# fatlipp/eacham

Measured on AMD Instinct MI355X. Metric: image-pairs matched/s + BA iters/s, 200-frame/50k-landmark synthetic, higher is better.
Workload: dtype i8; 1 GPU; S200 matching: 200 frames x 2000 kpts x 256-D, 19900 unordered pairs (both directions + mutual check); pairs_per_rank=19900, parallelism=pairs sharded over 1 GPU(s)

## Files before the change

### eacham_amd/csrc/context.hip

```cpp
#include "context.hpp"
#include <algorithm>

#include <cstdlib>
#include <cstring>
#include <dlfcn.h>
#include <new>

namespace eacham {

int ensure_workspace(eacham_ctx* ctx, size_t bytes) {
    if (bytes <= ctx->ws_bytes) return EACHAM_OK;
    if (ctx->ws) {
        EACHAM_HIP_TRY(ctx, hipStreamSynchronize(ctx->stream));
        EACHAM_HIP_TRY(ctx, hipFree(ctx->ws));
        ctx->ws = nullptr;
        ctx->ws_bytes = 0;
    }
    EACHAM_HIP_TRY(ctx, hipMalloc(&ctx->ws, bytes));
    ctx->ws_bytes = bytes;
    return EACHAM_OK;
}

int ensure_io(eacham_ctx* ctx, size_t bytes) {
    if (bytes <= ctx->io_bytes) return EACHAM_OK;
// ... 94 lines not shown
    f.dim = dim;
    f.ks = ks;
    f.ntiles = ntiles;
    ctx->ks_common = ks;
    ctx->kind_common = kind;
    ctx->wide_bytes_common = wide_bytes;
    ctx->frame_table_dirty = true;
    ctx->bits_table_dirty = true;
}

__global__ void gather_tiles_kernel(const FrameDev* __restrict__ frames, int n, int* __restrict__ used) {
    const int i = blockIdx.x * blockDim.x + threadIdx.x;
    if (i < n) used[i] = frames[i].meta ? frames[i].meta[1] : frames[i].ntiles;
}

int sync_frame_table(eacham_ctx* ctx) {
    if (!ctx->frame_table_dirty) return EACHAM_OK;
    int need = (int)ctx->frames.size();
    if (need + 1 > ctx->frame_table_cap) {
        if (ctx->frame_table_dev) {
            EACHAM_HIP_TRY(ctx, hipStreamSynchronize(ctx->stream));
            EACHAM_HIP_TRY(ctx, hipFree(ctx->frame_table_dev));
            ctx->frame_table_dev = nullptr;
        }
        int cap = need < 64 ? 64 : need * 2;
        EACHAM_HIP_TRY(ctx, hipMalloc((void**)&ctx->frame_table_dev, sizeof(FrameDev) * cap));
        ctx->frame_table_cap = cap;
    }
    std::vector<FrameDev> tab(need + 1);
    {
        FrameDev& e = tab[need];
        e.frag = nullptr; e.norm = nullptr; e.normb = nullptr; e.screen = nullptr;
        e.orig = ctx->flag_dev->standin_rows; e.pos = ctx->flag_dev->standin_rows; e.meta = ctx->flag_dev->standin_meta;
        e.n = 0; e.ntiles = 0; e.resident = 1;
    }
    for (int i = 0; i < need; ++i) {
        const FrameHost& f = ctx->frames[i];
        tab[i].frag = f.frag;
        tab[i].norm = f.norm;
        tab[i].normb = f.normb;
        tab[i].orig = f.orig;
        tab[i].pos = f.pos;
        tab[i].meta = f.meta;
        tab[i].screen = f.screen;
        tab[i].n = f.n < 0 ? 0 : f.n;
        tab[i].ntiles = f.n < 0 ? 0 : f.ntiles;
        tab[i].resident = f.n < 0 ? 0 : 1;
    }
    {
        EACHAM_HIP_TRY(ctx, hipMemcpyAsync(ctx->frame_table_dev, tab.data(), sizeof(FrameDev) * (need + 1),
                                           hipMemcpyHostToDevice, ctx->stream));
        int* used_dev = nullptr;
        if (need == 0) {
            ctx->frame_table_dirty = false;
            return EACHAM_OK;
        }
        EACHAM_HIP_TRY(ctx, hipMalloc((void**)&used_dev, sizeof(int) * need));
        gather_tiles_kernel<<<(need + 255) / 256, 256, 0, ctx->stream>>>(ctx->frame_table_dev, need, used_dev);
        std::vector<int> used(need);
        hipError_t e = hipMemcpyAsync(used.data(), used_dev, sizeof(int) * need, hipMemcpyDeviceToHost, ctx->stream);
        if (e == hipSuccess) e = hipStreamSynchronize(ctx->stream);
        (void)hipFree(used_dev);
        EACHAM_HIP_TRY(ctx, e);
        for (int i = 0; i < need; ++i) ctx->frames[i].tiles_used = used[i];
    }
    ctx->frame_table_dirty = false;
    return EACHAM_OK;
}

namespace {
typedef int (*roctx_push_t)(const char*);
typedef int (*roctx_pop_t)(void);
roctx_push_t g_roctx_push = nullptr;
roctx_pop_t g_roctx_pop = nullptr;
// ... 173 lines not shown
int eacham_clear_descriptors(eacham_ctx* ctx) {
    if (!ctx) return EACHAM_ERR_INVALID;
    std::lock_guard<std::mutex> lock(ctx->mu);
    (void)hipSetDevice(ctx->device);
    EACHAM_HIP_TRY(ctx, hipStreamSynchronize(ctx->stream));
    for (auto& f : ctx->frames) release_frame(f);
    ctx->frames.clear();
    ctx->ks_common = 0;
    ctx->kind_common = FRAME_INT8;
    ctx->wide_bytes_common = 0;
    ctx->frame_table_dirty = true;
    ctx->bits_table_dirty = true;
    return EACHAM_OK;
}

void eacham_ctx_destroy(eacham_ctx* ctx) {
    if (!ctx) return;
    (void)hipSetDevice(ctx->device);
    (void)hipStreamSynchronize(ctx->stream);
    for (auto& f : ctx->frames) release_frame(f);
    if (ctx->table16_dev) (void)hipFree(ctx->table16_dev);
    if (ctx->bits_table_dev) (void)hipFree((void*)ctx->bits_table_dev);
    if (ctx->frame_table_dev) (void)hipFree(ctx->frame_table_dev);
    if (ctx->flag_dev) (void)hipFree(ctx->flag_dev);
    if (ctx->pairs_safe) (void)hipFree(ctx->pairs_safe);
    if (ctx->ws) (void)hipFree(ctx->ws);
    if (ctx->io) (void)hipFree(ctx->io);
    if (ctx->io_host) (void)hipHostFree(ctx->io_host);
    for (auto& b : ctx->ba_pool) {
        if (b.dev) (void)hipFree(b.dev);
        if (b.pinned) (void)hipHostFree(b.pinned);
    }
    for (auto& sc : ctx->ba_scratch)
        if (sc.dev) (void)hipFree(sc.dev);
    for (auto& s : ctx->prof)
        for (auto& ev : s.events) {
            (void)hipEventDestroy(ev.first);
            (void)hipEventDestroy(ev.second);
        }
    for (hipEvent_t e : {ctx->ev_tile[0], ctx->ev_tile[1], ctx->ev_fin[0], ctx->ev_fin[1], ctx->ev_join})
        if (e) (void)hipEventDestroy(e);
    if (ctx->stream2) (void)hipStreamDestroy(ctx->stream2);
    (void)hipStreamDestroy(ctx->stream);
    delete ctx;
}

// ... 51 lines not shown
```

### eacham_amd/csrc/context.hpp

```cpp
#pragma once

#include <hip/hip_runtime.h>

#include <algorithm>
#include <cstdarg>
#include <cstddef>
#include <cstring>
#include <cstdint>
#include <cstdio>
#include <mutex>
#include <string>
#include <utility>
#include <vector>

#include "../../include/eacham_hip.h"
#include "io_layout.hpp"

namespace eacham {

enum FrameKind {
    FRAME_INT8 = 0,
    FRAME_F32 = 1,
    FRAME_BITS = 2,
    FRAME_BITS_WIDE = 3,
// ... 9 lines not shown
    int pad1[4];
    unsigned long long dot16[6];
    unsigned long long screen[3];
    int pad2[6];
};
static_assert(offsetof(FlagBlock, bad_pair) == 1 * sizeof(int) && offsetof(FlagBlock, standin_meta) == 8 * sizeof(int) &&
                  offsetof(FlagBlock, standin_rows) == 16 * sizeof(int) && offsetof(FlagBlock, colprune) == 32 * sizeof(int) &&
                  offsetof(FlagBlock, dot16) == 40 * sizeof(int) && offsetof(FlagBlock, screen) == 52 * sizeof(int) &&
                  sizeof(FlagBlock) == 64 * sizeof(int),
              "the block's words stay where the kernels and the debug calls have always found them");

struct FrameDev {
    const int4* frag;
    const int* norm;
    const int* normb;
    const int* orig;
    const int* pos;
    const int* meta;
    const int4* screen;
    int n;
    int ntiles;
    int resident;
};

struct FrameHost {
    int4* frag = nullptr;
    int* norm = nullptr;
    int* normb = nullptr;
    int* orig = nullptr;
    int* pos = nullptr;
    int* meta = nullptr;
    int4* screen = nullptr;
    unsigned* bits = nullptr;
    int n = -1;
    int dim = 0;
    int ks = 0;
    int ntiles = 0;
    int tiles_used = 0;
    void* img16 = nullptr;
    bool img16_ready = false;
    bool img16_bad = false;
    float img16_maxn = 0.0f;
};

struct BaBlock {
    void* dev = nullptr;
// ... 7 lines not shown
    size_t bytes = 0;
};

struct ProfileSlot {
    std::vector<std::pair<hipEvent_t, hipEvent_t>> events;
    size_t used = 0;
    int64_t launches = 0;
    double total_ms = 0.0;
};

}

struct eacham_ctx {
    int device = 0;
    hipStream_t stream = nullptr;
    hipStream_t stream2 = nullptr;
    hipEvent_t ev_tile[2] = {nullptr, nullptr}, ev_fin[2] = {nullptr, nullptr}, ev_join = nullptr;
    std::mutex mu;
    std::string err;

    std::vector<eacham::FrameHost> frames;
    eacham::FrameDev* frame_table_dev = nullptr;
    int frame_table_cap = 0;
    bool frame_table_dirty = true;
    eacham::FlagBlock* flag_dev = nullptr;
    int ks_common = 0;
    eacham::FrameKind kind_common = eacham::FRAME_INT8;
    const unsigned** bits_table_dev = nullptr;
    int bits_table_cap = 0;
    bool bits_table_dirty = true;
    int wide_bytes_common = 0;
    size_t wide_budget_bytes = 0;
    long long wide_debug[4] = {0, 0, 0, 0};
    void* table16_dev = nullptr;
    int table16_cap = 0;
    long long dot16_fallback_pairs = 0;

    void* ws = nullptr;
    size_t ws_bytes = 0;
    int2* pairs_safe = nullptr;
    int pairs_safe_cap = 0;
    void* io = nullptr;
    size_t io_bytes = 0;
    void* io_host = nullptr;
    size_t io_host_bytes = 0;

// ... 158 lines not shown
    }
};
struct LmedsLaunch {
    int kind, P;
    long long S, max_n;
    int score_grid;
    const long long *point_ptr, *sample_ptr;
    const double *a, *b, *K;
    bool has_K;
    const int* sample_idx;
    double* cand_models;
    int *n_models, *first, *sample_problem, *total, *scan_ws;
    float *cand_medians, *rows;
    double* models;
    float *medians, *thresholds;
    int* inliers;
    unsigned char* masks;
    int *winner, *n_candidates;
};
int lmeds_score_grid(long long cand_cap, long long max_n);
bool lmeds_needs_rows(long long max_n);
int lmeds_launch(eacham_ctx* ctx, hipStream_t st, const LmedsLaunch& L);
int sync_frame_table(eacham_ctx* ctx);
int sanitize_pairs(eacham_ctx* ctx, const int2* pairs_dev, int npairs, const int2** out);

int open_frame_slot(eacham_ctx* ctx, int frame_id, FrameKind kind, int n, int max_rows, int ks, int wide_bytes, FrameHost** slot);
void release_frame(FrameHost& f);
void commit_frame(eacham_ctx* ctx, FrameHost& f, FrameKind kind, int n, int dim, int ks, int ntiles, int wide_bytes);

int upload_frame_f32(eacham_ctx* ctx, int frame_id, const float* src_dev, int n, int dim);
int run_match_f32(eacham_ctx* ctx, const int2* pairs_dev, int npairs, double ratio, int min_dir, int min_mutual, int mode,
                  int* counts_dev, long long* offsets_dev, uint2* edges_dev, long long edge_cap, long long* total_dev,
                  int4* stats_dev);
struct MatchPlanF32 {
    int row_stride, wb_stride, wgs_per_pair;
    int batch;
    size_t off_rowres, off_colpart, off_matches, total;
};
MatchPlanF32 plan_match_f32(const eacham_ctx* ctx, int npairs);
int run_match_dot(eacham_ctx* ctx, const int2* pairs_dev, int npairs, float min_score, int min_dir, int min_mutual, int mode,
                  int* counts_dev, long long* offsets_dev, uint2* edges_dev, float* scores_dev, long long edge_cap,
                  long long* total_dev, int4* stats_dev);
void launch_match_tile_dot(eacham_ctx* ctx, const int2* pb, int nb, const MatchPlanF32& pl, int2* rr, int2* cp);
int launch_match_dot_tail(eacham_ctx* ctx, const MatchPlanF32& pl, const int2* pb, int nb, int first, bool is_last, int2* rr, int2* cp,
                          float min_score, int min_dir, int min_mutual, int mode, int* counts_dev, long long* offsets_dev,
                          uint2* edges_dev, float* scores_dev, long long edge_cap, long long* total_dev, int4* stats_dev);
// ... 30 lines not shown
```

### eacham_amd/csrc/matcher.hip

```cpp
#include "context.hpp"
#include "match_screen.hpp"
#include "match_tail.hpp"

#include <algorithm>
#include <climits>
#include <cstdlib>
#include <type_traits>

namespace eacham {

typedef int v4i __attribute__((ext_vector_type(4)));
typedef int v16i __attribute__((ext_vector_type(16)));
typedef const v4i __attribute__((address_space(1)))* gfrag_t;
typedef const int __attribute__((address_space(1)))* gint_t;

constexpr int PADH = 8350000;
constexpr int KEY_SHIFT = 7;
constexpr int KEY_MASK = (1 << KEY_SHIFT) - 1;
constexpr int CHUNK_TILES = 1 << KEY_SHIFT;
constexpr int MAX_ROWS = 16384;
constexpr int WG_THREADS = 256;
constexpr int WAVES = WG_THREADS / 64;
constexpr int MATCH_NSUB = 2;
constexpr int ROWS_PER_WAVE = 32 * MATCH_NSUB;
// ... 119 lines not shown
            const int x = min(max((int)src[(size_t)row * dim + k], 0), 255);
            code = screen::encode(x);
            const int m = screen::decode(code), d = x - screen::reconstruct(code);
            m2 += m * m;
            err += d * d;
        }
        codes[e] = (unsigned char)code;
    }
    uint32_t w[6];
    screen::pack32(codes, w);
    char* tb = image + (size_t)tile * SCREEN_TILE_BYTES + ks * SCREEN_STEP_BYTES;
    const int lane = 32 * h + r;
    *reinterpret_cast<v4i*>(tb + 16 * lane) = v4i{(int)w[0], (int)w[1], (int)w[2], (int)w[3]};
    *reinterpret_cast<int2*>(tb + 1024 + 8 * lane) = make_int2((int)w[4], (int)w[5]);
    if (m2) atomicAdd(&msq[j], m2);
    if (err) atomicAdd(&sr[j], err);
}
__global__ void finish_screen_kernel(int npad, const int* __restrict__ orig, int* __restrict__ msq, const int* __restrict__ sr, int* __restrict__ eb) {
    const int j = blockIdx.x * blockDim.x + threadIdx.x;
    if (j >= npad) return;
    const bool real_row = orig[j] >= 0;
    reinterpret_cast<float*>(msq)[j] = real_row ? 0.5f * (float)msq[j] : SCREEN_PAD;
    if (real_row) atomicMax(eb, sr[j]);
}

__device__ __forceinline__ unsigned vmed3(unsigned a, unsigned b, unsigned c) {
    unsigned d;
    asm("v_med3_u32 %0, %1, %2, %3" : "=v"(d) : "v"(a), "v"(b), "v"(c));
    return d;
}
__device__ __forceinline__ unsigned umin(unsigned a, unsigned b) { return a < b ? a : b; }
__device__ __forceinline__ unsigned umax(unsigned a, unsigned b) { return a > b ? a : b; }


__device__ __forceinline__ unsigned lds_addr(const void* p) {
    return (unsigned)(unsigned long long)(const __attribute__((address_space(3))) void*)p;
}
template <class V>
__device__ __forceinline__ void lds_read_frag(V& dst, unsigned addr, int offset_bytes) {
    asm volatile("ds_read_b128 %0, %1 offset:%2" : "=v"(dst) : "v"(addr), "n"(offset_bytes));
}

template <int KS>
__global__ __launch_bounds__(WG_THREADS, 2) void match_tile_kernel(
    const FrameDev* __restrict__ frames, const int2* __restrict__ pairs, int wgs_per_pair, int col_chunks,
    uint4* __restrict__ rowres, uint2* __restrict__ colpart, int wb_stride, int row_stride) {
// ... 543 lines not shown
        }
    }
}

typedef int v2i __attribute__((ext_vector_type(2)));
typedef int v6i __attribute__((ext_vector_type(6)));
typedef int v8i __attribute__((ext_vector_type(8)));
typedef float v4f __attribute__((ext_vector_type(4)));
typedef float v16f __attribute__((ext_vector_type(16)));
__device__ __forceinline__ void lds_read_frag64(v2i& dst, unsigned addr, int offset_bytes) {
    asm volatile("ds_read_b64 %0, %1 offset:%2" : "=v"(dst) : "v"(addr), "n"(offset_bytes));
}
__device__ __forceinline__ float fmin3(float a, float b, float c) {
    float d;
    asm("v_min3_f32 %0, %1, %2, %3" : "=v"(d) : "v"(a), "v"(b), "v"(c));
    return d;
}
template <int METRIC>
__device__ __forceinline__ bool ratio_pass(int d2_best, int d2_second, double ratio);
struct ScreenFrag { v4i lo; v2i hi; };
__device__ __forceinline__ v8i screen_operand(const ScreenFrag& f) { return v8i{f.lo[0], f.lo[1], f.lo[2], f.lo[3], f.hi[0], f.hi[1], 0, 0}; }

template <int METRIC>
__global__ __launch_bounds__(WG_THREADS, 3) void match_screen_kernel(const FrameDev* __restrict__ frames, const int2* __restrict__ pairs,
                                                                     int wgs_per_pair, uint4* __restrict__ rowres, int row_stride, double ratio,
                                                                     unsigned long long* __restrict__ openmask, int mask_stride) {
    constexpr int NSUB = 2, KS = SCREEN_KS;
    constexpr int TILE_V4 = SCREEN_TILE_BYTES / 16;
    constexpr int ROWS_WAVE = 32 * NSUB, ROWS_WG = WAVES * ROWS_WAVE;
    constexpr float BIGF = 3.0e38f;
    constexpr int SCALE = (int)0x82828282u;
    constexpr int NT = SCREEN_CALL_TILES, RING = 3 * NT;
    static_assert(NT == 2 && KS == 4 && NT * 32 == 64, "the waits of a call are counted for two tiles of four steps; wave 0 carries the constants of a call");
    __shared__ v4i sB[RING][TILE_V4];
    __shared__ __attribute__((aligned(16))) float sHb[RING][32];
    const int tid = threadIdx.x;
    const int lane = tid & 63;
    const int wave = __builtin_amdgcn_readfirstlane(tid >> 6);
    const int h = lane >> 5;
    const int rb = blockIdx.x % wgs_per_pair;
    const int p = blockIdx.x / wgs_per_pair;
    const int2 pr = pairs[p];
    const FrameDev A = frames[pr.x], B = frames[pr.y];
    const int A_even = ((gint_t)A.meta)[0], A_tiles = ((gint_t)A.meta)[1];
    const int T = ((gint_t)B.meta)[1];
    if (rb * (ROWS_WG / 32) >= A_tiles) return;
    const int wb = rb * WAVES + wave;
    const bool active = NSUB * wb < A_tiles;
    typedef const __attribute__((address_space(1))) char* gbytes_t;
    typedef const float __attribute__((address_space(1)))* gfloat_t;
    const gbytes_t Aimg = (gbytes_t)A.screen, Bimg = (gbytes_t)B.screen;
    const gfloat_t Am2 = (gfloat_t)(Aimg + (size_t)A.ntiles * SCREEN_TILE_BYTES), Bm2 = (gfloat_t)(Bimg + (size_t)B.ntiles * SCREEN_TILE_BYTES);
    const int wbc = active ? wb : 0;

    v6i a[NSUB][KS];
#pragma unroll
    for (int s = 0; s < NSUB; ++s)
#pragma unroll
        for (int ks = 0; ks < KS; ++ks) {
            const gbytes_t tb = Aimg + (size_t)(NSUB * wbc + s) * SCREEN_TILE_BYTES + ks * SCREEN_STEP_BYTES;
            const v4i lo = *(const v4i __attribute__((address_space(1)))*)(tb + 16 * lane);
            const v2i hi = *(const v2i __attribute__((address_space(1)))*)(tb + 1024 + 8 * lane);
            a[s][ks] = v6i{lo[0] ^ 0x20820820, lo[1] ^ 0x08208208, lo[2] ^ (int)0x82082082u, lo[3] ^ 0x20820820, hi[0] ^ 0x08208208, hi[1] ^ (int)0x82082082u};
        }
    float xm[2][NSUB][4];
#pragma unroll
    for (int q = 0; q < 2; ++q)
#pragma unroll
        for (int s = 0; s < NSUB; ++s)
#pragma unroll
            for (int g = 0; g < 4; ++g) xm[q][s][g] = BIGF;

    static_assert(TILE_V4 % 64 == 0, "a tile is a whole number of 1 KiB pieces");
    constexpr int PIECES = TILE_V4 / 64;
    static_assert((NT * PIECES) % WAVES == 0, "every wave stages the same number of pieces per call");
    constexpr int PPW = NT * PIECES / WAVES;
    const int TM = T - 1;
    unsigned stage_off = (unsigned)lane * 16u, hb_off = (unsigned)(lane & 31) * 4u;
    auto stage_piece = [&](int tile, int slot, int piece) {
        const gbytes_t base = Bimg + (size_t)min(tile, TM) * SCREEN_TILE_BYTES + piece * 1024;
        asm volatile("" : "+v"(stage_off));
        __builtin_amdgcn_global_load_lds((const __attribute__((address_space(1))) void*)(base + stage_off),
                                         (__attribute__((address_space(3))) void*)(&sB[slot][piece * 64]), 16, 0, 0);
    };
    auto load_hb = [&](int tile) {
        asm volatile("" : "+v"(hb_off));
        const gbytes_t row = reinterpret_cast<gbytes_t>(Bm2) + (size_t)128 * min(tile + (lane >> 5), TM);
        return *reinterpret_cast<gfloat_t>(row + hb_off);
    };
    float hb_new = 0.0f;
    if (T > 0) {
#pragma unroll
        for (int i = 0; i < ((2 * NT + 1) * PIECES + WAVES - 1) / WAVES; ++i) {
            const int idx = wave + WAVES * i;
            if (idx < (2 * NT + 1) * PIECES) stage_piece(idx / PIECES, idx / PIECES, idx % PIECES);
        }
        if (tid < 32 * (NT + 2)) sHb[tid >> 5][tid & 31] = Bm2[32 * min(tid >> 5, TM) + (tid & 31)];
        if (wave == 0) hb_new = load_hb(NT + 2);
    }
    __builtin_amdgcn_s_waitcnt(0);
    __syncthreads();

    typedef const v4f __attribute__((address_space(3)))* lds_v4f_t;
    lds_v4f_t hb_lane = (lds_v4f_t)(const __attribute__((address_space(3))) void*)&sHb[0][4 * h];
    asm volatile("" : "+v"(hb_lane));
    auto cinit_of = [&](int slot) {
        v16f c;
#pragma unroll
        for (int g = 0; g < 4; ++g) {
            const v4f q = hb_lane[8 * slot + 2 * g];
#pragma unroll
            for (int k = 0; k < 4; ++k) c[4 * g + k] = q[k];
        }
        return c;
    };
    int scale = SCALE;
    asm volatile("" : "+v"(scale));
    auto mfma = [&](const ScreenFrag& b, const v6i& q, const v16f& c) {
        const v8i q8 = __builtin_shufflevector(q, q, 0, 1, 2, 3, 4, 5, -1, -1);
        return __builtin_amdgcn_mfma_scale_f32_32x32x64_f8f6f4(screen_operand(b), q8, c, 2, 2, 0, scale, 0, scale);
    };
    v16f accA[NSUB], accB[NSUB];
#pragma unroll
// ... 103 lines not shown
        } else {
#pragma unroll
            for (int i = 0; i < PPW; ++i) stage(i);
        }
        asm volatile("s_waitcnt vmcnt(1)" : : : "memory");
        __builtin_amdgcn_s_barrier();
    };
    auto last = [&]() {
        if (active) {
#pragma unroll
            for (int idx = 0; idx < 32; ++idx) consume(accA, xm[0], idx);
        }
    };
    if (T > 0) {
        const int NC = (TM + 1) / 2;
        int c = 0;
        for (; c + 3 <= NC; c += 3) {
            call(std::integral_constant<int, 0>{}, NT * c);
            call(std::integral_constant<int, 1>{}, NT * (c + 1));
            call(std::integral_constant<int, 2>{}, NT * (c + 2));
        }
        if (c < NC) call(std::integral_constant<int, 0>{}, NT * c);
        if (c + 1 < NC) call(std::integral_constant<int, 1>{}, NT * (c + 1));
        asm volatile("s_waitcnt vmcnt(0)" : : : "memory");
        drain_lds();
        if (!(TM & 1)) last();
    }
    if (!active) return;
    const gint_t Asr = (gint_t)(Am2 + 32 * (size_t)A.ntiles);
    const int e_b = T > 0 ? ((gint_t)(Bm2 + 64 * (size_t)B.ntiles))[0] : 0;
    uint4* rr = rowres + (size_t)p * row_stride + ROWS_WAVE * wb;
    const int lane_t = (int)((lds16 - lds_addr(sBb)) >> 4), cl_t = lane_t & 31, h_t = lane_t >> 5;
    constexpr unsigned PAD_V = 2u * PADH;
    unsigned long long open_rows = 0;
#pragma unroll
    for (int s = 0; s < NSUB; ++s) {
        bool open = false;
        const int j = ROWS_WAVE * wb + 32 * s + cl_t;
        const float ma = Am2[j];
        float v1 = BIGF, v2 = BIGF;
#pragma unroll
        for (int q = 0; q < 2; ++q)
#pragma unroll
            for (int g = 0; g < 4; ++g) {
                const float mine = xm[q][s][g], other = __shfl_xor(mine, 32);
                v2 = fminf(v2, fmaxf(v1, mine)), v1 = fminf(v1, mine);
                v2 = fminf(v2, fmaxf(v1, other)), v1 = fminf(v1, other);
            }
        if (h_t == 0) {
            const bool real_row = ma < 0.5f * SCREEN_PAD;
            const bool real1 = real_row && v1 < 0.5f * SCREEN_PAD, real2 = real_row && v2 < 0.5f * SCREEN_PAD;
            const unsigned pa = NSUB * wb + s >= A_even ? 1u : 0u;
            const int s_a = Asr[j];
            const unsigned n1 = real1 ? (unsigned)(2.0f * (v1 + ma)) : 0u, u = real2 ? (unsigned)(2.0f * (v2 + ma)) : 0u;
            const unsigned w1 = real1 ? (unsigned)screen::lower_d2(n1, s_a, e_b) - pa + 2u : 0xffffffffu;
            const unsigned w2 = real2 ? (unsigned)screen::upper_d2(u, s_a, e_b) - pa + 2u : 0xffffffffu;
            rr[32 * s + cl_t] = make_uint4(w1, 0u, w2, real1 ? n1 : 0xffffffffu);
            open = NSUB * wb + s < A_tiles && w1 < PAD_V && (w2 >= PAD_V || ratio_pass<METRIC>((int)(w1 + pa) - 2, (int)(w2 + pa) - 2, ratio));
        }
        open_rows |= (__ballot(open) & 0xffffffffull) << (32 * s);
    }
    if (openmask && lane_t == 0) openmask[(size_t)p * mask_stride + wb] = open_rows;
}


constexpr int METRIC_L2 = 0, METRIC_HAMMING = 1;
template <int METRIC>
__device__ __forceinline__ bool ratio_pass(int d2_best, int d2_second, double ratio) {
    if (METRIC == METRIC_HAMMING) return d2_best >= 0 && d2_second >= 0 && (double)__fdiv_rn((float)d2_best, (float)d2_second) < ratio;
    float q = __fdiv_rn(__fsqrt_rn((float)d2_best), __fsqrt_rn((float)d2_second));
    return (double)q < ratio;
}

template <int METRIC>
__global__ __launch_bounds__(FIN_THREADS) void match_finalize_kernel(
    const FrameDev* __restrict__ frames, const int2* __restrict__ pairs,
    const uint4* __restrict__ rowres, const uint2* __restrict__ colpart, int col_chunks, int wb_stride,
    int row_stride, double ratio, int min_dir, int min_mutual, int mode,
    uint2* __restrict__ out_matches, int* __restrict__ counts, int4* __restrict__ stats) {
    extern __shared__ int smem[];
    const int tid = threadIdx.x;
    const int p = blockIdx.x;
    const int2 pr = pairs[p];
    const FrameDev A = frames[pr.x], B = frames[pr.y];
// ... 87 lines not shown
        bool ok = false;
        if (j < 32 * A_tiles && A.orig[j] >= 0) {
            const uint4 e = rowres[(size_t)p * row_stride + j];
            const unsigned pa = (j >> 5) >= A_even ? 1u : 0u;
            ok = e.x < PAD_V && (e.z >= PAD_V || ratio_pass<METRIC>((int)(e.x + pa) - 2, (int)(e.z + pa) - 2, ratio));
        }
        int total;
        const int rank = block_rank(ok, tid, s_wave, total);
        if (ok) cl[base + rank] = j;
        base += total;
    }
    const int groups = (base + VER_CANDS - 1) / VER_CANDS;
    if (tid == 0) {
        state[p] = make_int4(base, 0, 0, 0);
        s_item0 = groups ? atomicAdd(n_items, groups) : 0;
        if (tally) atomicAdd(&tally[1], (unsigned long long)base);
    }
    __syncthreads();
    for (int g = tid; g < groups; g += FIN_THREADS) items[s_item0 + g] = make_int2(p, g);
}

constexpr int LIST_WAVES = 16;
constexpr int OSCAN_THREADS = 1024;
__global__ __launch_bounds__(64 * LIST_WAVES) void match_opencount_kernel(const FrameDev* __restrict__ frames, const int2* __restrict__ pairs, int npairs,
                                                                          const unsigned long long* __restrict__ openmask, int mask_stride,
                                                                          int4* __restrict__ state, unsigned long long* __restrict__ tally) {
    __shared__ int s_open[LIST_WAVES], s_rows[LIST_WAVES];
    const int lane = threadIdx.x & 63;
    const int wave = __builtin_amdgcn_readfirstlane(threadIdx.x >> 6);
    const int p = blockIdx.x * LIST_WAVES + wave;
    int open = 0, rows = 0;
    if (p < npairs) {
        const FrameDev A = frames[pairs[p].x];
        rows = A.n;
        const int nwords = (A.meta[1] + 1) / 2;
        const unsigned long long* om = openmask + (size_t)p * mask_stride;
        for (int w = lane; w < nwords; w += 64) open += __popcll(om[w]);
#pragma unroll
        for (int d = 32; d >= 1; d >>= 1) open += __shfl_xor(open, d);
        if (lane == 0) ((int*)&state[p])[0] = open;
    }
    if (lane == 0) s_open[wave] = open, s_rows[wave] = rows;
    __syncthreads();
    if (threadIdx.x == 0) {
        unsigned long long r = 0, o = 0;
        for (int k = 0; k < LIST_WAVES; ++k) r += (unsigned long long)s_rows[k], o += (unsigned long long)s_open[k];
        atomicAdd(&tally[0], r);
        atomicAdd(&tally[1], o);
    }
}

template <bool MAX>
__device__ __forceinline__ int oscan_inclusive(int v, int* s_w , int* total) {
    const int lane = threadIdx.x & 63, wave = threadIdx.x >> 6;
#pragma unroll
    for (int d = 1; d < 64; d <<= 1) {
        const int u = __shfl_up(v, d);
        if (lane >= d) v = MAX ? max(v, u) : v + u;
// ... 46 lines not shown
        s_item0[tid] = it0, s_first[tid] = first, s_total[tid] = total;
        __syncthreads();
        for (int w = item0 + tid; w < item0 + chunk_items; w += OSCAN_THREADS) {
            int t = 0;
            for (int hi = OSCAN_THREADS; hi - t > 1;) {
                const int mid = (t + hi) >> 1;
                if (s_item0[mid] <= w) t = mid;
                else hi = mid;
            }
            const int k = w - s_item0[t];
            items[w] = make_int2(s_first[t] + k * width, min(width, s_total[t] - k * width));
        }
        seg0 = s_first[OSCAN_THREADS - 1];
        cand0 += chunk_cands;
        item0 += chunk_items;
        __syncthreads();
    }
    if (tid == 0) {
        *n_items = item0;
        atomicAdd(&tally[2], (unsigned long long)item0);
    }
}

__global__ __launch_bounds__(64 * LIST_WAVES) void match_openfill_kernel(const FrameDev* __restrict__ frames, const int2* __restrict__ pairs, int npairs,
                                                                         const unsigned long long* __restrict__ openmask, int mask_stride,
                                                                         const int4* __restrict__ state, uint2* __restrict__ cands) {
    const int lane = threadIdx.x & 63;
    const int wave = __builtin_amdgcn_readfirstlane(threadIdx.x >> 6);
    const int p = blockIdx.x * LIST_WAVES + wave;
    if (p >= npairs) return;
    const int4 st = state[p];
    if (st.x == 0) return;
    const int nwords = (frames[pairs[p].x].meta[1] + 1) / 2;
    const unsigned long long* om = openmask + (size_t)p * mask_stride;
    uint2* cl = cands + st.y;
    int base = 0;
    for (int w0 = 0; w0 < nwords; w0 += 64) {
        const unsigned long long mine = w0 + lane < nwords ? om[w0 + lane] : 0ull;
        const int nw = min(64, nwords - w0);
        for (int k = 0; k < nw; ++k) {
            const unsigned long long m = ((unsigned long long)(unsigned)__builtin_amdgcn_readlane((int)(mine >> 32), k) << 32) |
                                         (unsigned)__builtin_amdgcn_readlane((int)mine, k);
            if ((m >> lane) & 1) cl[base + __popcll(m & ((1ull << lane) - 1))] = make_uint2((unsigned)p, (unsigned)(64 * (w0 + k) + lane));
            base += __popcll(m);
        }
    }
}

constexpr int MAX_TILES = MAX_ROWS / 32;
constexpr int AITEM_SHARED = 1 << 16;
template <int METRIC, bool OPEN = false>
__global__ __launch_bounds__(FIN_THREADS) void match_rows2_kernel(
    const FrameDev* __restrict__ frames, const int2* __restrict__ pairs, const uint4* __restrict__ rowres, int row_stride, double ratio,
    int min_dir, int min_mutual, int mode, uint2* __restrict__ rowcand, int* __restrict__ candlist, int* __restrict__ bytile,
    int4* __restrict__ state, int4* __restrict__ aitems, int* __restrict__ n_aitems) {
    __shared__ int s_wave[FIN_THREADS / 64];
// ... 388 lines not shown
__global__ void compact_edges_kernel(const uint2* __restrict__ matches, const int* __restrict__ counts,
                                     const long long* __restrict__ offsets, int row_stride,
                                     uint2* __restrict__ edges, long long edge_cap) {
    const int p = blockIdx.x;
    const int n = counts[p];
    const long long off = offsets[p];
    for (int k = threadIdx.x; k < n; k += blockDim.x)
        if (off + k < edge_cap) edges[off + k] = matches[(size_t)p * row_stride + k];
}


static int ks_for_dim(int dim) {
    if (dim <= 0 || dim > 256) return 0;
    if (dim > 128) return 8;
    if (dim % 16) return 0;
    return dim <= 64 ? 2 : 4;
}

template <class F>
static void with_ks(int ks, F&& f) {
    if (ks == 2) f(std::integral_constant<int, 2>{});
    else if (ks == 4) f(std::integral_constant<int, 4>{});
    else f(std::integral_constant<int, 8>{});
}

static int upload_frame(eacham_ctx* ctx, int frame_id, const float* src_dev, int n, int dim, FrameKind kind = FRAME_INT8) {
    const int ks = ks_for_dim(dim);
    FrameHost* slot = nullptr;
    if (int rc = open_frame_slot(ctx, frame_id, kind, n, MAX_ROWS, ks, 0, &slot)) return rc;
    FrameHost& f = *slot;
    const int group_rows = 32 * GROUP_TILES;
    const int ntiles = n > 0 ? ((n + 31) / 32 + 1 + GROUP_TILES - 1) / GROUP_TILES * GROUP_TILES : 0;
    const int npad = ntiles * 32;
    {
        const size_t ints = (size_t)6 * npad + 2 + (kind == FRAME_BITS ? 6 + (size_t)8 * n : 0);
        EACHAM_HIP_TRY(ctx, hipMalloc((void**)&f.norm, ints * sizeof(int)));
        EACHAM_HIP_TRY(ctx, hipMemsetAsync(f.norm, 0, ints * sizeof(int), ctx->stream));
        f.normb = f.norm + npad;
        f.orig = f.norm + 2 * (size_t)npad;
        f.pos = f.norm + 3 * (size_t)npad;
        int* s2 = f.norm + 4 * (size_t)npad;
        int* s1 = f.norm + 5 * (size_t)npad;
        f.meta = f.norm + 6 * (size_t)npad;
        if (kind == FRAME_BITS) f.bits = (unsigned*)(f.norm + 6 * (size_t)npad + 8);
        if (npad > 0) {
            const size_t frag_bytes = (size_t)ntiles * ks * 64 * sizeof(int4);
// ... 150 lines not shown
    hipStream_t st1 = ctx->stream, st2 = pl.slots == 2 || npairs <= pl.batch ? ctx->stream2 : ctx->stream;
    EACHAM_HIP_TRY(ctx, hipEventRecord(ctx->ev_join, st1));
    EACHAM_HIP_TRY(ctx, hipStreamWaitEvent(st2, ctx->ev_join, 0));
    EACHAM_HIP_TRY(ctx, hipMemsetAsync(colprune_totals(ctx), 0, 2 * sizeof(unsigned long long), st2));
    const int form = ctx->match_sweep_form;
    const bool screen_sweep = !full_cols && (form == 0 || form == 3) && frames_have_screen(ctx);
    EACHAM_HIP_TRY(ctx, hipMemsetAsync(screen_tally(ctx), 0, 3 * sizeof(unsigned long long), screen_sweep ? st1 : st2));
    int b = 0;
    for (int first = 0, nb = 0; first < npairs; first += nb, ++b) {
        nb = next_batch(pl, b, first, npairs);
        const int slot = b % pl.slots;
        char* ws = (char*)ctx->ws + (size_t)slot * pl.slot_bytes;
        const int2* pb = pairs_dev + first;
        if (b >= pl.slots) EACHAM_HIP_TRY(ctx, hipStreamWaitEvent(st1, ctx->ev_fin[slot], 0));
        const bool bound_sweep = !full_cols && !screen_sweep && (form == 2 || ((form == 0 || form == 3) && ctx->ks_common <= 4));
        uint4* rowres = (uint4*)(ws + pl.off_rowres);
        int* n_pre = (int*)(ws + pl.off_nitems) + 8;
        const int vgrid = std::min(std::max(nb * pl.wgs_per_pair, 1), 512);
        {
            ProfileScope ps(ctx, EACHAM_KERNEL_MATCH_TILE, st1);
            with_ks(ctx->ks_common, [&](auto ks) {
                constexpr int KS = decltype(ks)::value;
                if (screen_sweep)
                    match_screen_kernel<METRIC><<<nb * pl.wgs_per_pair, WG_THREADS, 0, st1>>>(ctx->frame_table_dev, pb, pl.wgs_per_pair, rowres, pl.row_stride, ratio,
                                                                                          (unsigned long long*)(ws + pl.off_openmask), pl.mask_stride);
                else if (full_cols)
                    match_tile_kernel<KS><<<nb * pl.wgs_per_pair * pl.col_chunks, WG_THREADS, 0, st1>>>(
                        ctx->frame_table_dev, pb, pl.wgs_per_pair, pl.col_chunks, rowres, (uint2*)(ws + pl.off_colpart), pl.wb_stride, pl.row_stride);
                else if (bound_sweep)
                    match_sweep_kernel<KS, true><<<nb * pl.wgs_per_pair, WG_THREADS, 0, st1>>>(ctx->frame_table_dev, pb, pl.wgs_per_pair, rowres, pl.row_stride);
                else
                    match_sweep_kernel<KS, false><<<nb * pl.wgs_per_pair, WG_THREADS, 0, st1>>>(ctx->frame_table_dev, pb, pl.wgs_per_pair, rowres, pl.row_stride);
            });
        }
        if (screen_sweep) {
            ProfileScope ps(ctx, EACHAM_KERNEL_MATCH_FINALIZE, st1);
            uint2* cands = (uint2*)(ws + pl.off_rowcand);
            int4* state = (int4*)(ws + pl.off_state);
            int2* items = (int2*)(ws + pl.off_items);
            const unsigned long long* openmask = (const unsigned long long*)(ws + pl.off_openmask);
            const int lgrid = (nb + LIST_WAVES - 1) / LIST_WAVES;
            match_opencount_kernel<<<lgrid, 64 * LIST_WAVES, 0, st1>>>(ctx->frame_table_dev, pb, nb, openmask, pl.mask_stride, state, screen_tally(ctx));
            match_openscan_kernel<<<1, OSCAN_THREADS, 0, st1>>>(pb, nb, GATHER_WIDTH, state, items, n_pre, screen_tally(ctx));
            match_openfill_kernel<<<lgrid, 64 * LIST_WAVES, 0, st1>>>(ctx->frame_table_dev, pb, nb, openmask, pl.mask_stride, state, cands);
            const int ggrid = nb * ((pl.row_stride + GATHER_WIDTH - 1) / GATHER_WIDTH + 1);
            match_sweep_kernel<SCREEN_EXACT_KS, false, true><<<ggrid, WG_THREADS, 0, st1>>>(ctx->frame_table_dev, pb, 0, rowres, pl.row_stride,
                                                                                           GatherList<true>{cands, items, n_pre});
        }
        EACHAM_HIP_TRY(ctx, hipEventRecord(ctx->ev_tile[slot], st1));
        EACHAM_HIP_TRY(ctx, hipStreamWaitEvent(st2, ctx->ev_tile[slot], 0));
        int* cnt = counts_dev + first;
        {
            ProfileScope ps(ctx, EACHAM_KERNEL_MATCH_FINALIZE, st2);
            if (full_cols) {
                match_finalize_kernel<METRIC><<<nb, FIN_THREADS, fin_smem, st2>>>(
                    ctx->frame_table_dev, pb, rowres, (const uint2*)(ws + pl.off_colpart), pl.col_chunks, pl.wb_stride, pl.row_stride, ratio,
                    min_dir, min_mutual, mode, (uint2*)(ws + pl.off_matches), cnt, stats_dev ? stats_dev + first : nullptr);
            } else {
                uint2* rowcand = (uint2*)(ws + pl.off_rowcand);
                int* candlist = (int*)(ws + pl.off_candlist);
                uint2* colres = (uint2*)(ws + pl.off_colres);
                int4* state = (int4*)(ws + pl.off_state);
                int2* items = (int2*)(ws + pl.off_items);
                int* n_items = (int*)(ws + pl.off_nitems);
                int* n_aitems = n_items + 16;
                int* bytile = (int*)(ws + pl.off_bytile);
                int4* aitems = (int4*)(ws + pl.off_aitems);
// ... 308 lines not shown
int eacham_match_debug_screen_pair(eacham_ctx* ctx, int f1, int f2, uint32_t* n1, int32_t* l1, int32_t* u2, int cap) {
    return match_entry(ctx, [&]() -> int {
        if (!n1 || !l1 || !u2 || cap < 0) return ctx->fail(EACHAM_ERR_INVALID, "null output");
        const int32_t pr[2] = {f1, f2};
        int rc = check_pairs_host(ctx, pr, 1);
        if (rc) return rc;
        rc = check_integer_flag(ctx);
        if (rc) return rc;
        rc = sync_frame_table(ctx);
        if (rc) return rc;
        if (!frames_have_screen(ctx)) return ctx->fail(EACHAM_ERR_UNSUPPORTED, "the screen sweep needs int8 frames above 128-D");
        const FrameHost& A = ctx->frames[f1];
        if (cap < A.n) return ctx->fail(EACHAM_ERR_CAPACITY, "%d rows but capacity %d", A.n, cap);
        if (A.n == 0) return EACHAM_OK;
        MatchPlan pl = make_plan(ctx, 1, false);
        rc = ensure_workspace(ctx, pl.total);
        if (rc) return rc;
        IoStage io(ctx, ctx->stream);
        const auto h_pair = io.in<int2>(pr, 1);
        IoDev d;
        rc = io.upload(d);
        if (rc) return rc;
        uint4* rowres = (uint4*)((char*)ctx->ws + pl.off_rowres);
        match_screen_kernel<METRIC_L2><<<pl.wgs_per_pair, WG_THREADS, 0, ctx->stream>>>(ctx->frame_table_dev, d(h_pair), pl.wgs_per_pair, rowres, pl.row_stride, 0.0, nullptr, 0);
        EACHAM_HIP_TRY(ctx, hipGetLastError());
        rc = io.finish();
        if (rc) return rc;
        const int rows = 32 * A.tiles_used;
        std::vector<uint4> res((size_t)rows);
        std::vector<int> pos((size_t)A.n), meta(2);
        EACHAM_HIP_TRY(ctx, hipMemcpy(res.data(), rowres, sizeof(uint4) * res.size(), hipMemcpyDeviceToHost));
        EACHAM_HIP_TRY(ctx, hipMemcpy(pos.data(), A.pos, sizeof(int) * pos.size(), hipMemcpyDeviceToHost));
        EACHAM_HIP_TRY(ctx, hipMemcpy(meta.data(), A.meta, sizeof(int) * 2, hipMemcpyDeviceToHost));
        for (int q = 0; q < A.n; ++q) {
            const int j = pos[q];
            const uint4 e = res[j];
            const unsigned pa = (j >> 5) >= meta[0] ? 1u : 0u;
            n1[q] = e.w;
            l1[q] = e.x == 0xffffffffu ? -1 : (int32_t)(e.x + pa) - 2;
            u2[q] = e.z == 0xffffffffu ? -1 : (int32_t)(e.z + pa) - 2;
        }
        return EACHAM_OK;
    });
}

int eacham_match_pairs_directed(eacham_ctx* ctx, const int32_t* pairs, int npairs, double ratio, int32_t* counts,
                                int64_t* offsets, uint32_t* out_q, uint32_t* out_t, int64_t cap, int64_t* out_total) {
// ... 168 lines not shown
```

Baseline: 1.881 million image-pairs/s.

## Precompute per-frame screen records and restructure screen kernel prologue/epilogue loads

Adds a compact 32-byte ScreenRecord per frame, built on device when the frame table syncs. It holds the image pointer, tile counts and the B-side e value, so the screen kernel reads each frame with one scalar load instead of chasing meta pointers. The kernel also defers the XOR on the A fragments until after the staging waitcnt, issues the per-row ma/s_a loads early under a partial vmcnt wait, and collapses the per-subtile epilogue to a single store per lane. In exchange it adds another device table to allocate and keep in sync, plus hand-tuned waitcnt assumptions that are fragile.

```diff
diff --git a/eacham_amd/csrc/context.hip b/eacham_amd/csrc/context.hip
--- a/eacham_amd/csrc/context.hip
+++ b/eacham_amd/csrc/context.hip
@@ -140,9 +140,17 @@
             EACHAM_HIP_TRY(ctx, hipStreamSynchronize(ctx->stream));
             EACHAM_HIP_TRY(ctx, hipFree(ctx->frame_table_dev));
             ctx->frame_table_dev = nullptr;
+            ctx->frame_table_cap = 0;
+            if (ctx->screen_table_dev) EACHAM_HIP_TRY(ctx, hipFree(ctx->screen_table_dev));
+            ctx->screen_table_dev = nullptr;
         }
         int cap = need < 64 ? 64 : need * 2;
         EACHAM_HIP_TRY(ctx, hipMalloc((void**)&ctx->frame_table_dev, sizeof(FrameDev) * cap));
+        if (hipMalloc((void**)&ctx->screen_table_dev, sizeof(ScreenRecord) * cap) != hipSuccess) {
+            (void)hipFree(ctx->frame_table_dev);
+            ctx->frame_table_dev = nullptr;
+            return ctx->fail(EACHAM_ERR_HIP, "no memory for the frames' screen records");
+        }
         ctx->frame_table_cap = cap;
     }
     std::vector<FrameDev> tab(need + 1);
@@ -168,6 +176,7 @@
     {
         EACHAM_HIP_TRY(ctx, hipMemcpyAsync(ctx->frame_table_dev, tab.data(), sizeof(FrameDev) * (need + 1),
                                            hipMemcpyHostToDevice, ctx->stream));
+        if (int rc = write_screen_records(ctx, need + 1)) return rc;
         int* used_dev = nullptr;
         if (need == 0) {
             ctx->frame_table_dirty = false;
@@ -387,6 +396,7 @@
     if (ctx->table16_dev) (void)hipFree(ctx->table16_dev);
     if (ctx->bits_table_dev) (void)hipFree((void*)ctx->bits_table_dev);
     if (ctx->frame_table_dev) (void)hipFree(ctx->frame_table_dev);
+    if (ctx->screen_table_dev) (void)hipFree(ctx->screen_table_dev);
     if (ctx->flag_dev) (void)hipFree(ctx->flag_dev);
     if (ctx->pairs_safe) (void)hipFree(ctx->pairs_safe);
     if (ctx->ws) (void)hipFree(ctx->ws);
diff --git a/eacham_amd/csrc/context.hpp b/eacham_amd/csrc/context.hpp
--- a/eacham_amd/csrc/context.hpp
+++ b/eacham_amd/csrc/context.hpp
@@ -55,6 +55,16 @@
     int ntiles;
     int resident;
 };
+
+struct ScreenRecord {
+    const int4* image;
+    int ntiles;
+    int tiles_used;
+    int tiles_even;
+    int e;
+    int unused[2];
+};
+static_assert(sizeof(ScreenRecord) == 32, "one record is one aligned 32-byte load");
 
 struct FrameHost {
     int4* frag = nullptr;
@@ -108,6 +118,7 @@
     std::vector<eacham::FrameHost> frames;
     eacham::FrameDev* frame_table_dev = nullptr;
     int frame_table_cap = 0;
+    eacham::ScreenRecord* screen_table_dev = nullptr;
     bool frame_table_dirty = true;
     eacham::FlagBlock* flag_dev = nullptr;
     int ks_common = 0;
@@ -312,6 +323,7 @@
 bool lmeds_needs_rows(long long max_n);
 int lmeds_launch(eacham_ctx* ctx, hipStream_t st, const LmedsLaunch& L);
 int sync_frame_table(eacham_ctx* ctx);
+int write_screen_records(eacham_ctx* ctx, int n);
 int sanitize_pairs(eacham_ctx* ctx, const int2* pairs_dev, int npairs, const int2** out);
 
 int open_frame_slot(eacham_ctx* ctx, int frame_id, FrameKind kind, int n, int max_rows, int ks, int wide_bytes, FrameHost** slot);
diff --git a/eacham_amd/csrc/matcher.hip b/eacham_amd/csrc/matcher.hip
--- a/eacham_amd/csrc/matcher.hip
+++ b/eacham_amd/csrc/matcher.hip
@@ -165,6 +165,20 @@
     const bool real_row = orig[j] >= 0;
     reinterpret_cast<float*>(msq)[j] = real_row ? 0.5f * (float)msq[j] : SCREEN_PAD;
     if (real_row) atomicMax(eb, sr[j]);
+}
+__global__ void screen_records_kernel(const FrameDev* __restrict__ frames, int n, ScreenRecord* __restrict__ recs) {
+    const int i = blockIdx.x * blockDim.x + threadIdx.x;
+    if (i >= n) return;
+    const FrameDev f = frames[i];
+    ScreenRecord r = {nullptr, 0, 0, 0, 0, {0, 0}};
+    if (f.screen && f.ntiles > 0) {
+        r.image = f.screen;
+        r.ntiles = f.ntiles;
+        r.tiles_even = f.meta[0];
+        r.tiles_used = f.meta[1];
+        r.e = reinterpret_cast<const int*>(reinterpret_cast<const char*>(f.screen) + (size_t)f.ntiles * SCREEN_TILE_BYTES)[64 * (size_t)f.ntiles];
+    }
+    recs[i] = r;
 }
 
 __device__ __forceinline__ unsigned vmed3(unsigned a, unsigned b, unsigned c) {
@@ -754,7 +768,7 @@
 __device__ __forceinline__ v8i screen_operand(const ScreenFrag& f) { return v8i{f.lo[0], f.lo[1], f.lo[2], f.lo[3], f.hi[0], f.hi[1], 0, 0}; }
 
 template <int METRIC>
-__global__ __launch_bounds__(WG_THREADS, 3) void match_screen_kernel(const FrameDev* __restrict__ frames, const int2* __restrict__ pairs,
+__global__ __launch_bounds__(WG_THREADS, 3) void match_screen_kernel(const ScreenRecord* __restrict__ recs, const int2* __restrict__ pairs,
                                                                      int wgs_per_pair, uint4* __restrict__ rowres, int row_stride, double ratio,
                                                                      unsigned long long* __restrict__ openmask, int mask_stride) {
     constexpr int NSUB = 2, KS = SCREEN_KS;
@@ -773,27 +787,34 @@
     const int rb = blockIdx.x % wgs_per_pair;
     const int p = blockIdx.x / wgs_per_pair;
     const int2 pr = pairs[p];
-    const FrameDev A = frames[pr.x], B = frames[pr.y];
-    const int A_even = ((gint_t)A.meta)[0], A_tiles = ((gint_t)A.meta)[1];
-    const int T = ((gint_t)B.meta)[1];
+    v8i rec_a = *reinterpret_cast<const v8i*>(recs + pr.x), rec_b = *reinterpret_cast<const v8i*>(recs + pr.y);
+    asm volatile("" : "+s"(rec_a), "+s"(rec_b));
+    const auto record_of = [](const v8i& r) {
+        return ScreenRecord{reinterpret_cast<const int4*>(((unsigned long long)(unsigned)r[1] << 32) | (unsigned)r[0]), r[2], r[3], r[4], r[5], {0, 0}};
+    };
+    static_assert(offsetof(ScreenRecord, ntiles) == 8 && offsetof(ScreenRecord, tiles_used) == 12 && offsetof(ScreenRecord, tiles_even) == 16 &&
+                      offsetof(ScreenRecord, e) == 20, "record_of reads the record's words by number");
+    const ScreenRecord A = record_of(rec_a), B = record_of(rec_b);
+    const int A_even = A.tiles_even, A_tiles = A.tiles_used;
+    const int T = B.tiles_used;
     if (rb * (ROWS_WG / 32) >= A_tiles) return;
     const int wb = rb * WAVES + wave;
     const bool active = NSUB * wb < A_tiles;
     typedef const __attribute__((address_space(1))) char* gbytes_t;
     typedef const float __attribute__((address_space(1)))* gfloat_t;
-    const gbytes_t Aimg = (gbytes_t)A.screen, Bimg = (gbytes_t)B.screen;
+    const gbytes_t Aimg = (gbytes_t)A.image, Bimg = (gbytes_t)B.image;
     const gfloat_t Am2 = (gfloat_t)(Aimg + (size_t)A.ntiles * SCREEN_TILE_BYTES), Bm2 = (gfloat_t)(Bimg + (size_t)B.ntiles * SCREEN_TILE_BYTES);
     const int wbc = active ? wb : 0;
 
-    v6i a[NSUB][KS];
+    v4i alo[NSUB][KS];
+    v2i ahi[NSUB][KS];
 #pragma unroll
     for (int s = 0; s < NSUB; ++s)
 #pragma unroll
         for (int ks = 0; ks < KS; ++ks) {
             const gbytes_t tb = Aimg + (size_t)(NSUB * wbc + s) * SCREEN_TILE_BYTES + ks * SCREEN_STEP_BYTES;
-            const v4i lo = *(const v4i __attribute__((address_space(1)))*)(tb + 16 * lane);
-            const v2i hi = *(const v2i __attribute__((address_space(1)))*)(tb + 1024 + 8 * lane);
-            a[s][ks] = v6i{lo[0] ^ 0x20820820, lo[1] ^ 0x08208208, lo[2] ^ (int)0x82082082u, lo[3] ^ 0x20820820, hi[0] ^ 0x08208208, hi[1] ^ (int)0x82082082u};
+            alo[s][ks] = *(const v4i __attribute__((address_space(1)))*)(tb + 16 * lane);
+            ahi[s][ks] = *(const v2i __attribute__((address_space(1)))*)(tb + 1024 + 8 * lane);
         }
     float xm[2][NSUB][4];
 #pragma unroll
@@ -820,17 +841,28 @@
         const gbytes_t row = reinterpret_cast<gbytes_t>(Bm2) + (size_t)128 * min(tile + (lane >> 5), TM);
         return *reinterpret_cast<gfloat_t>(row + hb_off);
     };
-    float hb_new = 0.0f;
+    float hb_new = 0.0f, hb_first = 0.0f;
     if (T > 0) {
 #pragma unroll
         for (int i = 0; i < ((2 * NT + 1) * PIECES + WAVES - 1) / WAVES; ++i) {
             const int idx = wave + WAVES * i;
             if (idx < (2 * NT + 1) * PIECES) stage_piece(idx / PIECES, idx / PIECES, idx % PIECES);
         }
-        if (tid < 32 * (NT + 2)) sHb[tid >> 5][tid & 31] = Bm2[32 * min(tid >> 5, TM) + (tid & 31)];
+        if (tid < 32 * (NT + 2)) hb_first = Bm2[32 * min(tid >> 5, TM) + (tid & 31)];
         if (wave == 0) hb_new = load_hb(NT + 2);
     }
     __builtin_amdgcn_s_waitcnt(0);
+    if (T > 0 && tid < 32 * (NT + 2)) sHb[tid >> 5][tid & 31] = hb_first;
+    v6i a[NSUB][KS];
+#pragma unroll
+    for (int s = 0; s < NSUB; ++s)
+#pragma unroll
+        for (int ks = 0; ks < KS; ++ks) {
+            v4i lo = alo[s][ks];
+            v2i hi = ahi[s][ks];
+            asm volatile("" : "+v"(lo), "+v"(hi));
+            a[s][ks] = v6i{lo[0] ^ 0x20820820, lo[1] ^ 0x08208208, lo[2] ^ (int)0x82082082u, lo[3] ^ 0x20820820, hi[0] ^ 0x08208208, hi[1] ^ (int)0x82082082u};
+        }
     __syncthreads();
 
     typedef const v4f __attribute__((address_space(3)))* lds_v4f_t;
@@ -980,44 +1012,51 @@
         }
         if (c < NC) call(std::integral_constant<int, 0>{}, NT * c);
         if (c + 1 < NC) call(std::integral_constant<int, 1>{}, NT * (c + 1));
-        asm volatile("s_waitcnt vmcnt(0)" : : : "memory");
+    }
+    const int lane_t = (int)((lds16 - lds_addr(sBb)) >> 4), h_t = lane_t >> 5;
+    const gint_t Asr = (gint_t)(Am2 + 32 * (size_t)A.ntiles);
+    float ma = 0.0f;
+    int s_a = 0;
+    if (active) {
+        const int j = ROWS_WAVE * wb + lane_t;
+        ma = Am2[j];
+        s_a = Asr[j];
+    }
+    if (T > 0) {
+        if (active) asm volatile("s_waitcnt vmcnt(2)" : : : "memory");
+        else asm volatile("s_waitcnt vmcnt(0)" : : : "memory");
         drain_lds();
         if (!(TM & 1)) last();
     }
     if (!active) return;
-    const gint_t Asr = (gint_t)(Am2 + 32 * (size_t)A.ntiles);
-    const int e_b = T > 0 ? ((gint_t)(Bm2 + 64 * (size_t)B.ntiles))[0] : 0;
+    asm volatile("" : "+v"(ma), "+v"(s_a));
+    const int e_b = B.e;
     uint4* rr = rowres + (size_t)p * row_stride + ROWS_WAVE * wb;
-    const int lane_t = (int)((lds16 - lds_addr(sBb)) >> 4), cl_t = lane_t & 31, h_t = lane_t >> 5;
     constexpr unsigned PAD_V = 2u * PADH;
-    unsigned long long open_rows = 0;
+    float v1 = BIGF, v2 = BIGF;
 #pragma unroll
     for (int s = 0; s < NSUB; ++s) {
-        bool open = false;
-        const int j = ROWS_WAVE * wb + 32 * s + cl_t;
-        const float ma = Am2[j];
-        float v1 = BIGF, v2 = BIGF;
+        float m1 = BIGF, m2 = BIGF;
 #pragma unroll
         for (int q = 0; q < 2; ++q)
 #pragma unroll
             for (int g = 0; g < 4; ++g) {
                 const float mine = xm[q][s][g], other = __shfl_xor(mine, 32);
-                v2 = fminf(v2, fmaxf(v1, mine)), v1 = fminf(v1, mine);
-                v2 = fminf(v2, fmaxf(v1, other)), v1 = fminf(v1, other);
+                m2 = fminf(m2, fmaxf(m1, mine)), m1 = fminf(m1, mine);
+                m2 = fminf(m2, fmaxf(m1, other)), m1 = fminf(m1, other);
             }
-        if (h_t == 0) {
-            const bool real_row = ma < 0.5f * SCREEN_PAD;
-            const bool real1 = real_row && v1 < 0.5f * SCREEN_PAD, real2 = real_row && v2 < 0.5f * SCREEN_PAD;
-            const unsigned pa = NSUB * wb + s >= A_even ? 1u : 0u;
-            const int s_a = Asr[j];
-            const unsigned n1 = real1 ? (unsigned)(2.0f * (v1 + ma)) : 0u, u = real2 ? (unsigned)(2.0f * (v2 + ma)) : 0u;
-            const unsigned w1 = real1 ? (unsigned)screen::lower_d2(n1, s_a, e_b) - pa + 2u : 0xffffffffu;
-            const unsigned w2 = real2 ? (unsigned)screen::upper_d2(u, s_a, e_b) - pa + 2u : 0xffffffffu;
-            rr[32 * s + cl_t] = make_uint4(w1, 0u, w2, real1 ? n1 : 0xffffffffu);
-            open = NSUB * wb + s < A_tiles && w1 < PAD_V && (w2 >= PAD_V || ratio_pass<METRIC>((int)(w1 + pa) - 2, (int)(w2 + pa) - 2, ratio));
-        }
-        open_rows |= (__ballot(open) & 0xffffffffull) << (32 * s);
-    }
+        if (s == 0 || h_t == s) v1 = m1, v2 = m2;
+    }
+    const bool real_row = ma < 0.5f * SCREEN_PAD;
+    const bool real1 = real_row && v1 < 0.5f * SCREEN_PAD, real2 = real_row && v2 < 0.5f * SCREEN_PAD;
+    const int tile_t = NSUB * wb + h_t;
+    const unsigned pa = tile_t >= A_even ? 1u : 0u;
+    const unsigned n1 = real1 ? (unsigned)(2.0f * (v1 + ma)) : 0u, u = real2 ? (unsigned)(2.0f * (v2 + ma)) : 0u;
+    const unsigned w1 = real1 ? (unsigned)screen::lower_d2(n1, s_a, e_b) - pa + 2u : 0xffffffffu;
+    const unsigned w2 = real2 ? (unsigned)screen::upper_d2(u, s_a, e_b) - pa + 2u : 0xffffffffu;
+    rr[lane_t] = make_uint4(w1, 0u, w2, real1 ? n1 : 0xffffffffu);
+    const bool open = tile_t < A_tiles && w1 < PAD_V && (w2 >= PAD_V || ratio_pass<METRIC>((int)(w1 + pa) - 2, (int)(w2 + pa) - 2, ratio));
+    const unsigned long long open_rows = __ballot(open);
     if (openmask && lane_t == 0) openmask[(size_t)p * mask_stride + wb] = open_rows;
 }
 
@@ -1151,7 +1190,7 @@
 
 constexpr int LIST_WAVES = 16;
 constexpr int OSCAN_THREADS = 1024;
-__global__ __launch_bounds__(64 * LIST_WAVES) void match_opencount_kernel(const FrameDev* __restrict__ frames, const int2* __restrict__ pairs, int npairs,
+__global__ __launch_bounds__(64 * LIST_WAVES) void match_opencount_kernel(const FrameDev* __restrict__ frames, const ScreenRecord* __restrict__ recs, const int2* __restrict__ pairs, int npairs,
                                                                           const unsigned long long* __restrict__ openmask, int mask_stride,
                                                                           int4* __restrict__ state, unsigned long long* __restrict__ tally) {
     __shared__ int s_open[LIST_WAVES], s_rows[LIST_WAVES];
@@ -1160,9 +1199,9 @@
     const int p = blockIdx.x * LIST_WAVES + wave;
     int open = 0, rows = 0;
     if (p < npairs) {
-        const FrameDev A = frames[pairs[p].x];
-        rows = A.n;
-        const int nwords = (A.meta[1] + 1) / 2;
+        const int fa = pairs[p].x;
+        rows = frames[fa].n;
+        const int nwords = (recs[fa].tiles_used + 1) / 2;
         const unsigned long long* om = openmask + (size_t)p * mask_stride;
         for (int w = lane; w < nwords; w += 64) open += __popcll(om[w]);
 #pragma unroll
@@ -1255,7 +1294,7 @@
     }
 }
 
-__global__ __launch_bounds__(64 * LIST_WAVES) void match_openfill_kernel(const FrameDev* __restrict__ frames, const int2* __restrict__ pairs, int npairs,
+__global__ __launch_bounds__(64 * LIST_WAVES) void match_openfill_kernel(const ScreenRecord* __restrict__ recs, const int2* __restrict__ pairs, int npairs,
                                                                          const unsigned long long* __restrict__ openmask, int mask_stride,
                                                                          const int4* __restrict__ state, uint2* __restrict__ cands) {
     const int lane = threadIdx.x & 63;
@@ -1264,7 +1303,7 @@
     if (p >= npairs) return;
     const int4 st = state[p];
     if (st.x == 0) return;
-    const int nwords = (frames[pairs[p].x].meta[1] + 1) / 2;
+    const int nwords = (recs[pairs[p].x].tiles_used + 1) / 2;
     const unsigned long long* om = openmask + (size_t)p * mask_stride;
     uint2* cl = cands + st.y;
     int base = 0;
@@ -1699,6 +1738,13 @@
     if (ks == 2) f(std::integral_constant<int, 2>{});
     else if (ks == 4) f(std::integral_constant<int, 4>{});
     else f(std::integral_constant<int, 8>{});
+}
+
+int write_screen_records(eacham_ctx* ctx, int n) {
+    if (n <= 0) return EACHAM_OK;
+    screen_records_kernel<<<(n + 255) / 256, 256, 0, ctx->stream>>>(ctx->frame_table_dev, n, ctx->screen_table_dev);
+    EACHAM_HIP_TRY(ctx, hipGetLastError());
+    return EACHAM_OK;
 }
 
 static int upload_frame(eacham_ctx* ctx, int frame_id, const float* src_dev, int n, int dim, FrameKind kind = FRAME_INT8) {
@@ -1895,7 +1941,7 @@
             with_ks(ctx->ks_common, [&](auto ks) {
                 constexpr int KS = decltype(ks)::value;
                 if (screen_sweep)
-                    match_screen_kernel<METRIC><<<nb * pl.wgs_per_pair, WG_THREADS, 0, st1>>>(ctx->frame_table_dev, pb, pl.wgs_per_pair, rowres, pl.row_stride, ratio,
+                    match_screen_kernel<METRIC><<<nb * pl.wgs_per_pair, WG_THREADS, 0, st1>>>(ctx->screen_table_dev, pb, pl.wgs_per_pair, rowres, pl.row_stride, ratio,
                                                                                           (unsigned long long*)(ws + pl.off_openmask), pl.mask_stride);
                 else if (full_cols)
                     match_tile_kernel<KS><<<nb * pl.wgs_per_pair * pl.col_chunks, WG_THREADS, 0, st1>>>(
@@ -1913,9 +1959,9 @@
             int2* items = (int2*)(ws + pl.off_items);
             const unsigned long long* openmask = (const unsigned long long*)(ws + pl.off_openmask);
             const int lgrid = (nb + LIST_WAVES - 1) / LIST_WAVES;
-            match_opencount_kernel<<<lgrid, 64 * LIST_WAVES, 0, st1>>>(ctx->frame_table_dev, pb, nb, openmask, pl.mask_stride, state, screen_tally(ctx));
+            match_opencount_kernel<<<lgrid, 64 * LIST_WAVES, 0, st1>>>(ctx->frame_table_dev, ctx->screen_table_dev, pb, nb, openmask, pl.mask_stride, state, screen_tally(ctx));
             match_openscan_kernel<<<1, OSCAN_THREADS, 0, st1>>>(pb, nb, GATHER_WIDTH, state, items, n_pre, screen_tally(ctx));
-            match_openfill_kernel<<<lgrid, 64 * LIST_WAVES, 0, st1>>>(ctx->frame_table_dev, pb, nb, openmask, pl.mask_stride, state, cands);
+            match_openfill_kernel<<<lgrid, 64 * LIST_WAVES, 0, st1>>>(ctx->screen_table_dev, pb, nb, openmask, pl.mask_stride, state, cands);
             const int ggrid = nb * ((pl.row_stride + GATHER_WIDTH - 1) / GATHER_WIDTH + 1);
             match_sweep_kernel<SCREEN_EXACT_KS, false, true><<<ggrid, WG_THREADS, 0, st1>>>(ctx->frame_table_dev, pb, 0, rowres, pl.row_stride,
                                                                                            GatherList<true>{cands, items, n_pre});
@@ -2270,7 +2316,7 @@
         rc = io.upload(d);
         if (rc) return rc;
         uint4* rowres = (uint4*)((char*)ctx->ws + pl.off_rowres);
-        match_screen_kernel<METRIC_L2><<<pl.wgs_per_pair, WG_THREADS, 0, ctx->stream>>>(ctx->frame_table_dev, d(h_pair), pl.wgs_per_pair, rowres, pl.row_stride, 0.0, nullptr, 0);
+        match_screen_kernel<METRIC_L2><<<pl.wgs_per_pair, WG_THREADS, 0, ctx->stream>>>(ctx->screen_table_dev, d(h_pair), pl.wgs_per_pair, rowres, pl.row_stride, 0.0, nullptr, 0);
         EACHAM_HIP_TRY(ctx, hipGetLastError());
         rc = io.finish();
         if (rc) return rc;
```

Result: no change. 1.898 million image-pairs/s (median of 6 runs) (+0.9%).
